# akamiru/bce

Hardware: AMD Instinct MI355X
Metric: MB/s compressed (higher is better)
Workload: dtype u8/u32 integer

## Files before the change

### bce_amd/csrc/api.hip

```cpp
#include <condition_variable>
#include <functional>
#include <mutex>
#include <thread>
#include <new>
#include <utility>

#include "bce_cost.h"
#include "common.h"
#include "host_coder.h"
#include "scan_coder.h"

#include <dlfcn.h>
#include <errno.h>
#include <fcntl.h>
#include <sys/file.h>
#include <sys/mman.h>
#include <sys/stat.h>
#include <unistd.h>

using namespace bce;

#ifndef K3_BATCH_MID
#define K3_BATCH_MID 8u
#endif
// ... 938 lines not shown
  c->stats.t_enum = c->stats.k3_ms * 1e-3;
  if (gate_timing)
    fprintf(stderr, "gate: ctx %p waited %.1f ms, held %.1f ms of %.1f ms from encode's start to its last flush queued (K3 %.1f ms, model %.1f ms, %llu flushes); coders' tail %.1f ms\n",
            (void *)c, c->gate_wait_s * 1e3, c->gate_held_s * 1e3, (t_gpu_done - t_enc0) * 1e3, c->stats.k3_ms, c->stats.t_model * 1e3,
            (unsigned long long)c->stats.flushes, (now_s() - t_gpu_done) * 1e3);
  return BCE_HIP_OK;
}

static int encode_body(bce_hip_ctx *c);
int bce_hip_encode(bce_hip_ctx *c) { return gate_on_error(c, bce_guarded(c, [&] { return encode_body(c); })); }
static int encode_body(bce_hip_ctx *c) {
  BCE_TRY(check_stage(c, 3));
  PhaseScope phase(c, 3);
  const double t_enc0 = now_s();
  BCE_TRY(encode_start(c));
  Enumeration e(c, [&](uint64_t nsym) { return flush_symbols(c, nsym); });
  BCE_TRY(e.run());
  return encode_end(c, e.ctl, t_enc0);
}

static bool early_enum_applies(const bce_hip_ctx *c) {
  const char *e = getenv("BCE_HIP_EARLY_ENUM");
  return !(e && e[0] == '0' && !e[1]) && k1_two_halves(c);
}
static uint32_t early_round_limit(uint32_t h) {
  uint32_t limit = 8u * h;
  if (const char *e = getenv("BCE_HIP_EARLY_CAP")) { const unsigned long v = strtoul(e, nullptr, 10); if (v < limit) limit = (uint32_t)v; }
  return limit;
}
static int compress_early_body(bce_hip_ctx *c) {
  BCE_TRY(check_stage(c, 1));
  BCE_HIP_TRY(c, hipSetDevice(c->device));
  c->stage = 1; c->enum_active = false;
  uint32_t h = 0;
  double t0 = now_s();
  PhaseScope phase(c, 1);
  {
    RoctxRange range("bce K1 first sort + provisional BWT");
    BCE_TRY(k1_first_sort(c, &h));
    BCE_TRY(k1_provisional_bwt(c));
  }
  double t_bwt = now_s() - t0;
  t0 = now_s();
  phase.set(2);
  {
    RoctxRange range("bce K2 planes + rank directory (provisional)");
    BCE_TRY(k2_build_planes(c));
  }
  double t_planes = now_s() - t0;
  uint32_t zeros0[8];
  memcpy(zeros0, c->zeros, sizeof zeros0);

  phase.set(6);
  const double t_enc0 = now_s();
  BCE_TRY(encode_start(c));
  Enumeration e(c, [&](uint64_t nsym) { return flush_symbols(c, nsym); });
  e.round_limit = early_round_limit(h);
  BCE_TRY(e.run());
  if (!e.paused) { gate_release(c); c->gate_lent = false; }
  const uint32_t paused_at = c->round;
  const uint64_t early_syms = c->stats.symbols;
  const double t_early = now_s() - t_enc0;

  t0 = now_s();
  {
    RoctxRange range("bce K1 second half + BWT");
    BCE_TRY(k1_finish(c));
    BCE_TRY(k1_final_bwt(c, c->k1_first_final));
  }
  t_bwt += now_s() - t0;
  if (!c->k1_first_final) {
    t0 = now_s();
    RoctxRange range("bce K2 planes + rank directory");
    BCE_TRY(k2_build_planes(c));
    t_planes += now_s() - t0;
    if (memcmp(zeros0, c->zeros, sizeof zeros0) != 0) {
      snprintf(c->err, sizeof c->err, "early rounds: the planes of the provisional and of the final BWT differ in their zero counts");
      return BCE_HIP_E_INTERNAL;
    }
  }
  c->stats.t_bwt = t_bwt;
  c->stats.t_planes = t_planes;
  if (getenv("BCE_HIP_EARLY_TRACE"))
    fprintf(stderr, "early: h %u limit %u %s at round %u (%s) symbols %llu rounds %.2f ms k1_finish+planes %.2f ms first_sort_final %d\n", h, e.round_limit,
            e.paused ? "paused" : "finished", paused_at, !e.paused ? "end" : (paused_at >= e.round_limit ? "limit" : "tail due"),
            (unsigned long long)early_syms, t_early * 1e3, (now_s() - t_enc0 - t_early) * 1e3, (int)c->k1_first_final);
  phase.set(3);
  if (e.paused) {
    e.round_limit = Enumeration::kNoLimit;
    BCE_TRY(e.run());
  }
  return encode_end(c, e.ctl, t_enc0);
}
static int compress_early(bce_hip_ctx *c) {
  const int rc = gate_on_error(c, bce_guarded(c, [&] { return compress_early_body(c); }));
  if (rc != BCE_HIP_OK && c) { c->stage = c->text_loaded ? 1 : 0; c->enum_active = false; c->k1_valid = false; }
  return rc;
}

static int scan_body(bce_hip_ctx *c, uint8_t *config288, double *result_bytes);
int bce_hip_scan(bce_hip_ctx *c, uint8_t config288[BCE_HIP_CONFIG_BYTES], double result_bytes[9]) {
  const int r = bce_guarded(c, [&] { return scan_body(c, config288, result_bytes); });
  if (c) gate_release(c);
  return r;
}
static int scan_body(bce_hip_ctx *c, uint8_t *config288, double *result_bytes) {
  BCE_TRY(check_stage(c, 3));
  if (!config288) return BCE_HIP_E_ARG;
  const double t_begin = now_s();
  gate_acquire(c);
  BCE_HIP_TRY(c, hipSetDevice(c->device));
  c->coder->drain();
  c->scan_mode = true;
  PhaseScope phase(c, 3);
  struct Reset { bce_hip_ctx *c; ~Reset() { c->scan_mode = false; } } reset{c};
  BCE_TRY(k4_prepare(c));
  BCE_TRY(k3_begin(c));
  c->stats.t_coder = 0;
  ScanSet coders;
  struct PinnedWords {
    uint32_t *p = nullptr; size_t cap = 0;
    ~PinnedWords() { if (p) (void)hipHostFree(p); }
    int ensure(size_t words) {
      if (words <= cap) return 0;
      if (p) { (void)hipHostFree(p); p = nullptr; cap = 0; }
      if (hipHostMalloc(reinterpret_cast<void **>(&p), words * 4, hipHostMallocDefault) != hipSuccess) { p = nullptr; return 1; }
      cap = words;
      return 0;
    }
  } host;
  double t_copy = 0, t_record = 0, t_pin = 0;
  auto consume = [&](uint64_t nsym) -> int {
    if (nsym) {
      const double tp0 = now_s();
      if (host.ensure((size_t)nsym > (size_t)c->sym_cap ? (size_t)nsym : (size_t)c->sym_cap)) return BCE_HIP_E_NOMEM;
      const double tc0 = now_s();
      t_pin += tc0 - tp0;
      BCE_HIP_TRY(c, hipMemcpyAsync(host.p, c->scanrec.p, (size_t)nsym * 4, hipMemcpyDeviceToHost, c->stream));
      BCE_HIP_TRY(c, hipStreamSynchronize(c->stream));
      t_copy += now_s() - tc0;
      std::vector<ScanSpan> spans[8];
      for (int p = 0; p < 8; ++p)
        for (const RunEntry &e : c->run_log[p]) spans[p].push_back(ScanSpan{e.start, e.count});
      const double t0 = now_s();
      coders.consume(host.p, spans);
      c->stats.t_coder += now_s() - t0;
      t_record += now_s() - t0;
    }
    return k3_reset_symbols(c);
  };
  c->stats.flushes = 0; c->stats.symbols = 0;
  Enumeration e(c, [&](uint64_t nsym) { c->stats.flushes++; c->stats.symbols += nsym; return consume(nsym); });
  BCE_TRY(e.run());
  c->stats.rounds = e.ctl.done_round;
  c->stats.nodes = e.ctl.nodes_total;
  c->enum_active = false;
  uint8_t init[9][32];
  memset(init, 0, sizeof init);
  double res[9];
  const double tf0 = now_s();
  coders.flush(init, res);
  c->stats.t_coder += now_s() - tf0;
  if (getenv("BCE_HIP_SCAN_DEBUG"))
    fprintf(stderr, "scan: %llu symbols in %llu batches: pinned buffer %.3f s, device-to-host copies %.3f s, recording %.3f s, optimisation %.3f s on %u host threads; K3 %.1f ms; %.3f s since entry\n",
            (unsigned long long)c->stats.symbols, (unsigned long long)c->stats.flushes, t_pin, t_copy, t_record, now_s() - tf0, coders.threads(), c->stats.k3_ms, now_s() - t_begin);
  if (result_bytes) memcpy(result_bytes, res, sizeof res);
  memcpy(config288, init, BCE_HIP_CONFIG_BYTES);
  if (getenv("BCE_HIP_SCAN_DEBUG")) {
    const double t0 = now_s();
// ... 291 lines not shown
```

### bce_amd/csrc/common.h

```cpp
#pragma once
#include <hip/hip_runtime.h>
#include <stdint.h>
#include <stdio.h>
#include <stdlib.h>
#include <string.h>

#include <atomic>
#include <chrono>
#include <condition_variable>
#include <exception>
#include <new>
#include <memory>
#include <mutex>
#include <thread>
#include <vector>

#include <sys/mman.h>

#include "../../include/bce_hip.h"
#include "bce_core.h"
#include "host_coder.h"

namespace bce {

// ... 51 lines not shown
  if (base == MAP_FAILED) return nullptr;
  char *q = reinterpret_cast<char *>((reinterpret_cast<uintptr_t>(base) + two_mb - 1) & ~(uintptr_t)(two_mb - 1));
  const size_t head = (size_t)(q - static_cast<char *>(base));
  if (head) (void)munmap(base, head);
  if (two_mb - head) (void)munmap(q + used, two_mb - head);
  (void)madvise(q, used, MADV_DONTFORK);
  static const bool no_thp = getenv("BCE_HIP_NO_THP") != nullptr;
  if (!no_thp) (void)madvise(q, used, MADV_HUGEPAGE);
  return q;
}
inline void reg_map_settle(void *q, size_t bytes) { (void)madvise(q, (bytes + 4095) & ~(size_t)4095, MADV_NOHUGEPAGE); }
inline void huge_unmap(void *q, size_t bytes) { if (q) (void)munmap(q, (bytes + 4095) & ~(size_t)4095); }
inline size_t slot_map_bytes(size_t cap) { return (cap * 8 + 16 + 4095) & ~(size_t)4095; }
inline void slot_free_host(FlushSlot &s, uint32_t *unmaps = nullptr) {
  if (s.h_out) {
    if (s.registered) {
      if (s.ev_copy) (void)hipEventSynchronize(s.ev_copy);
      (void)hipHostUnregister(s.h_out);
      huge_unmap(s.h_out, slot_map_bytes(s.cap));
      if (unmaps) ++*unmaps;
    } else (void)hipHostFree(s.h_out);
  }
  s.h_out = nullptr; s.cap = 0; s.registered = false;
}

struct RunEntry { uint64_t start; uint32_t count; uint32_t round; };

namespace qb {
enum Id {
  cnt_res,
  cnt_pat, cnt_off, cnt_out,
  loc_res,
  loc_lo, loc_cnt, loc_drop, loc_start, loc_lin, loc_bsum,
  loc_key0, loc_key1, loc_val0, loc_val1,
  loc_pat, loc_off, loc_hits, loc_pos,
  mat_res,
  mat_bsum,
  mat_qry, mat_len, mat_pos,
  rep_res,
  rep_bsum,
  rep_lcp,
  par_res,
  par_exit, par_entry, par_flag,
  par_bsum, par_bcnt,
  par_hpre,
  par_off, par_loff,
  par_ops, par_lits, par_out,
  count
};
}

}

struct bce_hip_ctx {
  int device = 0;
  hipStream_t stream = nullptr;
  hipStream_t copy_stream = nullptr;
  hipStream_t k4_stream = nullptr;
  hipEvent_t ev_k3_batch = nullptr;
  hipEvent_t ev_k4_done[2] = {nullptr, nullptr};
  bool overlap = false;
  bool gated = true;
  bool gate_held = false;
  bool gate_lent = false;
  double gate_t0 = 0, gate_wait_s = 0, gate_held_s = 0;
  uint32_t flush_seq = 0;
  hipEvent_t copy_busy = nullptr;
  hipEvent_t ev0 = nullptr, ev1 = nullptr, ev_k4 = nullptr;
  char err[256] = {0};

  uint32_t n = 0;
  int stage = 0;
  int phase = 0;
  uint32_t offset = 0;
  uint8_t config[9][32];
  bce::PlaneCfg cfg[8];
  uint32_t zeros[8] = {0};
  bool k1_unique = false;
  bool k1_valid = false;
  int sa_res = 0;
  int k1_res = 0;
  uint32_t k1_h = 0;
  bool k1_first_final = false;
  uint32_t dbg_dfs_budget = 0, dbg_no_dfs = 0, dbg_no_tail = 0, dbg_no_skip = 0, dbg_no_small = 0, dbg_step_small = 0, dbg_no_fused = 0, dbg_no_local = 0, dbg_capp_div = 0, dbg_local_from = 0, dbg_local_budget = 0, dbg_tail_round = 0;
  uint32_t dbg_dec_budget = 0;
  uint32_t dbg_oom = 0;
  uint64_t sym_cap_user = 0;
  bool sync_flush = false;
  bce_hip_progress_fn progress = nullptr;
  void *progress_user = nullptr;

  bce::DevBuf text, bwt;
  bce::DevBuf sa[2], key[2], rank, k2, nrk, act[2];
  bce::DevBuf khi[2], dl[4], kflag, actv[2];
  bce::DevBuf rs_hist, blk;
  bce::DevBuf ptmp[2];
  bce::DevBuf gran;
  uint32_t ngran = 0;
  bce::DevBuf nlist[2];
  uint32_t capL[2] = {0, 0};
  bce::DevBuf dlist[2][8];
  int dec_part = 0;
  bce::DevBuf ctl, tilecnt, tileoff, runs;
  bce::DevBuf smwords;
  size_t k3_groups = 0;
  uint32_t k3_count2_grid = 0;
  bce::DevBuf k3tw, k3grp;
  bce::DevBuf dfs;
  bce::DevBuf truns;
  void *h_truns = nullptr;
  bce::DevBuf skey[2], sval[2], sout, sesc;
  bce::DevBuf skey_alt, sesc_alt, rs_hist_k4;
  uint64_t sym_cap = 0;
  bool estimate_mode = false;
  bool scan_mode = false;
  bce::DevBuf scanrec;
  bce::DevBuf stat, dcfg, k4w;
  bce::DevBuf cost_acc, cost_runs;
  bce::DevBuf crc_tab;
  uint32_t crc_tab_grid = 0;
  bce::DevBuf cmp_res;
  bce::DevBuf qbuf[bce::qb::count];
  bce::DevBuf hook[3];
  bool crc_const_ready = false;
  bool text_loaded = false;
  uint32_t stat_off[8] = {0};
  bool model_hook = false;

  void *h_ctl = nullptr, *h_runs = nullptr;
  void *h_small = nullptr;
  void *h_big = nullptr;
  size_t h_big_cap = 0;
  uint32_t dec_restarts = 0;
  uint64_t dec_list_grows = 0, dec_split_rounds = 0;
  uint32_t reg_maps = 0, reg_unmaps = 0;
  bool h_big_registered = false;
  void *dec_pin[3] = {nullptr, nullptr, nullptr};
  size_t dec_pin_cap[3] = {0, 0, 0};
  bce::FlushSlot slot[3];
  int slot_next = 0;

  uint32_t round = 0;
  bool enum_active = false;
  std::vector<bce::RunEntry> run_log[8];

  bce::HostCoder *coder = nullptr;
  bce_hip_stats stats;
  std::mutex stage_mu;
  std::condition_variable stage_cv;
  int stage_state = 1;
  double alloc_s = 0, pin_s = 0;
  uint64_t alloc_bytes = 0, pin_bytes = 0;
  uint32_t alloc_calls = 0, pin_calls = 0;
};

namespace bce {

inline double now_s() {
  return std::chrono::duration<double>(std::chrono::steady_clock::now().time_since_epoch()).count();
}

void *big_host_alloc(size_t bytes, int device, bool *registered);
void big_host_free(bce_hip_ctx *c, void *p, size_t bytes, bool registered);

inline int set_err(bce_hip_ctx *c, hipError_t e, const char *what, int line) {
  snprintf(c->err, sizeof c->err, "%s:%d: %s", what, line, hipGetErrorString(e));
// ... 187 lines not shown
```

### bce_amd/csrc/k1_bwt.hip

```cpp
#include <stdlib.h>

#include <utility>

#include "common.h"
#include "scan_util.h"

namespace bce {

#ifndef K1_ACT_TENTHS
#define K1_ACT_TENTHS 6
#endif

constexpr int K1_T = 256;

constexpr uint32_t K1_MAXB = 1024;
struct K1Plan { uint32_t nb, per_block; };
static K1Plan k1_plan(uint32_t n) {
  const uint32_t chunk = 2048;
  uint32_t chunks = (uint32_t)(((uint64_t)n + chunk - 1) / chunk);
  if (!chunks) chunks = 1;
  uint32_t nb = chunks < K1_MAXB ? chunks : K1_MAXB;
  uint32_t cpb = (chunks + nb - 1) / nb;
  nb = (chunks + cpb - 1) / cpb;
  return {nb, cpb * chunk};
// ... 283 lines not shown
  auto rerank = [&](const uint32_t *k1s, const uint32_t *k2s, const uint32_t *sa) -> int {
    BCE_HIP_TRY(c, hipMemsetAsync(scalars, 0, 4, c->stream));
    hipLaunchKernelGGL(k1_heads_kernel, dim3(pl.nb), dim3(K1_T), 0, c->stream, k1s, k2s, n, pl.per_block, nrk,
                       blockmax, scalars);
    hipLaunchKernelGGL(k1_apply_kernel, dim3(pl.nb), dim3(K1_T), 0, c->stream, nrk, blockmax, n, pl.per_block, sa,
                       rank);
    BCE_TRY(read_back(c, &groups, scalars, 4));
    return BCE_HIP_OK;
  };
  BCE_TRY(rerank(key[res], nullptr, val[res]));
  const uint32_t bits = ceil_log2(n);
  const uint32_t dg = 9;
  uint64_t h = sentinel ? 3 : 4;
  uint32_t *act[2] = {c->act[0].as<uint32_t>(), c->act[1].as<uint32_t>()};
  uint32_t m = n;
  bool have_list = false;
  auto build_active = [&](const uint32_t *nrk_in, const uint32_t *src, uint32_t cnt, uint32_t *out) -> int {
    const K1Plan ap = k1_plan(cnt);
    hipLaunchKernelGGL(k1_active_kernel<0>, dim3(ap.nb), dim3(K1_T), 0, c->stream, nrk_in, src, cnt, ap.per_block, ap.nb,
                       blockmax, out, scalars + 2);
    hipLaunchKernelGGL(k1_active_kernel<1>, dim3(ap.nb), dim3(K1_T), 0, c->stream, nrk_in, src, cnt, ap.per_block, ap.nb,
                       blockmax, out, scalars + 2);
    BCE_TRY(read_back(c, &m, scalars + 2, 4));
    return BCE_HIP_OK;
  };
  const bool trace = getenv("BCE_K1_TRACE") != nullptr;
  double t_prev = now_s();
  if (trace) fprintf(stderr, "k1 %p: start n %u groups %u\n", (void *)c, n, groups);
  while (groups < n && h < n) {
    if (trace) { const double t = now_s(); fprintf(stderr, "k1 %p: h %llu groups %u m %u list %d (+%.2f ms)\n", (void *)c, (unsigned long long)h, groups, m, (int)have_list, (t - t_prev) * 1e3); t_prev = t; }
    if (!have_list && (uint64_t)(n - groups) * 10 < (uint64_t)n * K1_ACT_TENTHS + 10) {
      BCE_TRY(build_active(nrk, nullptr, n, act[0]));
      have_list = true;
      if (m == 0) break;
    }
    if (have_list && (uint64_t)m * 10 < (uint64_t)n * K1_ACT_TENTHS) {
      const uint32_t *A = act[0];
      uint32_t *ki[2] = {key[0], key[1]};
      uint32_t *vi[2] = {val[res ^ 1], k2};
      const uint32_t ga = grid_for(m);
      hipLaunchKernelGGL(k1_act_gather_kernel, dim3(ga), dim3(K1_T), 0, c->stream, A, val[res], rank, n, m, (uint32_t)h,
                         ki[0], vi[0]);
      int r1 = 0;
      BCE_TRY(radix_sort_pairs(c, ki, vi, m, 0, bits, &r1, dg));
      uint32_t *kj[2] = {ki[r1 ^ 1], ki[r1]};
      uint32_t *vj[2] = {vi[r1], vi[r1 ^ 1]};
      hipLaunchKernelGGL(k1_act_group_kernel, dim3(ga), dim3(K1_T), 0, c->stream, vj[0], rank, m, kj[0]);
      int r2 = 0;
      BCE_TRY(radix_sort_pairs(c, kj, vj, m, 0, bits, &r2, dg));
      const K1Plan ap = k1_plan(m);
      hipLaunchKernelGGL(k1_act_heads_kernel, dim3(ap.nb), dim3(K1_T), 0, c->stream, A, vj[r2], kj[r2], rank, n, m,
                         (uint32_t)h, ap.per_block, val[res], nrk, blockmax);
      hipLaunchKernelGGL(k1_act_apply_kernel, dim3(ap.nb), dim3(K1_T), 0, c->stream, nrk, blockmax, m, ap.per_block,
                         vj[r2], rank);
      BCE_TRY(build_active(nrk, A, m, act[1]));
      std::swap(act[0], act[1]);
      h <<= 1;
      c->stats.sort_rounds++;
      if (m == 0) break;
      continue;
    }
    uint32_t *ki[2] = {key[res ^ 1], key[res]};
    uint32_t *vi[2] = {val[res ^ 1], val[res]};
    hipLaunchKernelGGL(k1_gather_prev_kernel, dim3(g), dim3(K1_T), 0, c->stream, val[res], rank, n, (uint32_t)h,
                       ki[0], vi[0]);
    int r2 = 0;
    BCE_TRY(radix_sort_pairs(c, ki, vi, n, 0, bits, &r2, dg));
    uint32_t *sk = ki[r2], *ssa = vi[r2];
    hipLaunchKernelGGL(k1_gather_next_kernel, dim3(g), dim3(K1_T), 0, c->stream, ssa, rank, n, (uint32_t)h, k2);
    BCE_TRY(rerank(sk, k2, ssa));
    res = (ssa == val[0]) ? 0 : 1;
    h <<= 1;
    c->stats.sort_rounds++;
    have_list = false;
  }
  c->k1_unique = (groups >= n) || (have_list && m == 0);
  c->sa_res = res;
  return BCE_HIP_OK;
}


constexpr uint32_t K1_SLOT = 0x7FFFFFFFu, K1_HEAD = 0x80000000u;
constexpr uint32_t K1_SC_HIST = 16, K1_SC_CODE = 16 + 256;
constexpr uint8_t KF_HEAD = 1, KF_KEEP = 2, KF_DEFER = 4;

__global__ __launch_bounds__(K1_T) void k1_bytehist_kernel(const uint8_t *__restrict__ T, uint32_t n, uint32_t *__restrict__ hist) {
  __shared__ uint32_t lh[256];
  lh[threadIdx.x] = 0;
  __syncthreads();
  for (uint64_t i = (uint64_t)blockIdx.x * K1_T + threadIdx.x; i < n; i += (uint64_t)gridDim.x * K1_T) atomicAdd(&lh[T[i]], 1u);
  __syncthreads();
  if (lh[threadIdx.x]) atomicAdd(&hist[threadIdx.x], lh[threadIdx.x]);
}

constexpr int K1I_E = 8;
__global__ __launch_bounds__(K1_T) void k1_init64_kernel(const uint8_t *__restrict__ T, uint32_t m, uint32_t nbytes,
                                                         const uint16_t *__restrict__ code, uint32_t bits, uint32_t nsym,
                                                         uint32_t *__restrict__ lo, uint32_t *__restrict__ hi, uint32_t *__restrict__ val) {
  __shared__ uint16_t sym[K1_T * K1I_E + 16];
  __shared__ uint16_t lut[256];
  lut[threadIdx.x] = code[threadIdx.x];
  __syncthreads();
  const uint64_t base = (uint64_t)blockIdx.x * (K1_T * K1I_E);
  for (uint32_t i = threadIdx.x; i < K1_T * K1I_E + 16; i += K1_T) {
    uint64_t q = base + i;
    if (q >= m) q %= m;
    sym[i] = q < nbytes ? lut[T[q]] : (uint16_t)0;
  }
  __syncthreads();
#pragma unroll
  for (int e = 0; e < K1I_E; ++e) {
    const uint32_t o = (uint32_t)e * K1_T + threadIdx.x;
    const uint64_t p = base + o;
    if (p < m) {
      uint64_t k = 0;
      for (uint32_t b = 0; b < nsym; ++b) k = (k << bits) | sym[o + b];
      lo[p] = (uint32_t)k;
      hi[p] = (uint32_t)(k >> 32);
      val[p] = (uint32_t)p;
    }
  }
}

constexpr int SEG_T = 1024;
constexpr int SEG_CH = 2048;
constexpr int SEG_CAP = 2048;
constexpr int SEG_W = SEG_CH + SEG_CAP;
constexpr int SEG_HW = SEG_W + SEG_CAP;

__device__ __forceinline__ int seg_prev_bit(const uint64_t *b, int pos, int lo_limit) {
  int wi = pos >> 6;
  uint64_t word = b[wi] & (~0ull >> (63 - (pos & 63)));
  const int wl = lo_limit >> 6;
  while (word == 0 && wi > wl) { --wi; word = b[wi]; }
  if (!word) return -1;
  const int r = wi * 64 + 63 - __clzll((long long)word);
  return r >= lo_limit ? r : -1;
}
__device__ __forceinline__ int seg_next_bit(const uint64_t *b, int pos, int hi_limit) {
  int wi = pos >> 6;
  uint64_t word = (pos & 63) == 63 ? 0ull : (b[wi] & (~0ull << ((pos & 63) + 1)));
  const int wh = hi_limit >> 6;
  while (word == 0 && wi < wh) { ++wi; word = b[wi]; }
  if (!word) return -1;
  const int r = wi * 64 + __ffsll((long long)word) - 1;
  return r <= hi_limit ? r : -1;
}

__global__ __launch_bounds__(SEG_T) void k1_seg_sort_kernel(const uint32_t *__restrict__ A, const uint32_t *__restrict__ V, uint32_t m, uint32_t *__restrict__ sa,
                                                            const uint32_t *__restrict__ rank, uint32_t n, uint32_t h,
                                                            uint32_t *__restrict__ nr, uint32_t *__restrict__ vs,
                                                            uint8_t *__restrict__ flag, uint32_t *__restrict__ ndefer) {
  __shared__ uint64_t hb[SEG_HW / 64 + 1];
  __shared__ uint64_t nbits[SEG_W / 64 + 1];
  __shared__ __attribute__((aligned(16))) uint32_t K[SEG_W];
  __shared__ uint32_t S[SEG_W], SL[SEG_W];
  __shared__ uint32_t s_defer;
  __shared__ int s_cntw;
  const uint32_t tid = threadIdx.x, lane = tid & 63u;
  const int64_t base = (int64_t)blockIdx.x * SEG_CH;
  if (tid == 0) { s_defer = 0; hb[SEG_HW / 64] = 0; nbits[SEG_W / 64] = 0; }
#pragma unroll
  for (int it = 0; it < SEG_HW / SEG_T; ++it) {
    const int u = it * SEG_T + (int)tid;
    const int64_t i = base - SEG_CAP + u;
    uint32_t a = 0;
    bool hd = false;
    if (i >= 0) {
      if (i < (int64_t)m) { a = A[i]; hd = (a & K1_HEAD) != 0u; }
      else hd = true;
    }
    const uint64_t bal = __ballot(hd);
    if (lane == 0) hb[u >> 6] = bal;
    if (u >= SEG_CAP) SL[u - SEG_CAP] = a & K1_SLOT;
  }
  __syncthreads();
  if (tid == 0) {
    const int e = seg_next_bit(hb, SEG_CAP + SEG_CH - 1, SEG_HW - 1);
    const int cw = (e < 0 ? SEG_HW : e) - SEG_CAP;
    s_cntw = cw > SEG_CH ? cw : SEG_CH;
  }
  __syncthreads();
  const int cntw = s_cntw;
  constexpr int EPT = SEG_W / SEG_T;
  uint32_t k2[EPT], sfx[EPT];
  int gs[EPT], ge[EPT];
  bool mine[EPT];
  uint32_t ndef = 0;
#pragma unroll
  for (int it = 0; it < EPT; ++it) {
    const int w = it * SEG_T + (int)tid, u = w + SEG_CAP;
    const int64_t i = base + w;
    mine[it] = false; gs[it] = 0; ge[it] = 0; k2[it] = 0; sfx[it] = 0;
    if (w < cntw && i < (int64_t)m) {
      const int g0 = seg_prev_bit(hb, u, u - SEG_CAP + 1);
      bool big = g0 < 0;
      int g1 = -1;
      if (!big) {
        const int lim = g0 + SEG_CAP < SEG_HW - 1 ? g0 + SEG_CAP : SEG_HW - 1;
        g1 = seg_next_bit(hb, u, lim);
        big = g1 < 0;
      }
      if (big) {
// ... 137 lines not shown
      hbase += htot;
    }
  }
}

__global__ __launch_bounds__(K1_T) void k1_big_gather_kernel(const uint32_t *__restrict__ idx, const uint32_t *__restrict__ gid,
                                                             const uint32_t *__restrict__ V, const uint32_t *__restrict__ rank,
                                                             uint32_t n, uint32_t nd, uint32_t h, uint32_t rbits,
                                                             uint32_t *__restrict__ lo, uint32_t *__restrict__ hi, uint32_t *__restrict__ val) {
  for (uint64_t j = (uint64_t)blockIdx.x * K1_T + threadIdx.x; j < nd; j += (uint64_t)gridDim.x * K1_T) {
    const uint32_t p = V[idx[j]];
    uint64_t q = (uint64_t)p + h;
    if (q >= n) q -= n;
    const uint64_t key = ((uint64_t)gid[j] << rbits) | rank[q];
    lo[j] = (uint32_t)key;
    hi[j] = (uint32_t)(key >> 32);
    val[j] = p;
  }
}
__global__ __launch_bounds__(K1_T) void k1_big_heads_kernel(const uint32_t *__restrict__ slots, const uint32_t *__restrict__ lo,
                                                            const uint32_t *__restrict__ hi, const uint32_t *__restrict__ val,
                                                            uint32_t nd, uint32_t per_block, uint32_t *__restrict__ sa,
                                                            uint32_t *__restrict__ nrk, uint32_t *__restrict__ blockmax) {
  const uint64_t beg = (uint64_t)blockIdx.x * per_block;
  uint64_t end = beg + per_block;
  if (end > nd) end = nd;
  uint32_t mx = 0;
  for (uint64_t j = beg + threadIdx.x; j < end; j += K1_T) {
    const uint32_t slot = slots[j];
    sa[slot] = val[j];
    const bool head = j == 0 || lo[j] != lo[j - 1] || hi[j] != hi[j - 1];
    nrk[j] = head ? slot : 0u;
    if (head) mx = slot;
  }
  mx = block_reduce_max<K1_T>(mx);
  if (threadIdx.x == 0) blockmax[blockIdx.x] = mx;
}

__global__ __launch_bounds__(K1_T) void k1_defer_flags_kernel(const uint32_t *__restrict__ nrk, const uint32_t *__restrict__ idx,
                                                              const uint32_t *__restrict__ sorted, uint32_t nd,
                                                              uint8_t *__restrict__ flag, uint32_t *__restrict__ vs) {
  for (uint64_t j = (uint64_t)blockIdx.x * K1_T + threadIdx.x; j < nd; j += (uint64_t)gridDim.x * K1_T) {
    const bool hd = j == 0 || nrk[j] != 0u;
    const bool nx = j + 1 >= nd || nrk[j + 1] != 0u;
    const uint32_t i = idx[j];
    flag[i] = (uint8_t)(KF_DEFER | (hd ? KF_HEAD : 0) | ((hd && nx) ? 0 : KF_KEEP));
    vs[i] = sorted[j];
  }
}

static uint32_t k1_part_min() {
  static const uint32_t part_min = getenv("BCE_K1_PART_MIN") ? (uint32_t)strtoul(getenv("BCE_K1_PART_MIN"), nullptr, 10) : K1_PART_MIN;
  return part_min;
}

struct K1View {
  bce_hip_ctx *c;
  uint32_t n, g;
  K1Plan pl;
  uint32_t *blockmax, *scalars;
  uint32_t *rank, *k2, *nrk;
  uint8_t *flag;
  uint32_t *lo[2], *hi[2], *val[2];
  bool trace;
  double t_prev;
  explicit K1View(bce_hip_ctx *ctx, uint32_t n_) : c(ctx), n(n_), g(grid_for(n_)), pl(k1_plan(n_)) {
    blockmax = c->blk.as<uint32_t>();
    scalars = blockmax + K1_MAXB;
    rank = c->rank.as<uint32_t>(); k2 = c->k2.as<uint32_t>(); nrk = c->nrk.as<uint32_t>();
    flag = c->kflag.as<uint8_t>();
    for (int i = 0; i < 2; ++i) { lo[i] = c->key[i].as<uint32_t>(); hi[i] = c->khi[i].as<uint32_t>(); val[i] = c->sa[i].as<uint32_t>(); }
    trace = getenv("BCE_K1_TRACE") != nullptr;
    t_prev = now_s();
  }
  void lap(const char *what, uint64_t h, uint32_t m, uint32_t nd) {
    if (!trace) return;
    (void)hipStreamSynchronize(c->stream);
    const double t = now_s();
    fprintf(stderr, "k1 %p: %-10s h %llu active %u deferred %u (+%.2f ms)\n", (void *)c, what, (unsigned long long)h, m, nd, (t - t_prev) * 1e3);
    t_prev = t;
  }
};

static int k1_first_sort_wide(bce_hip_ctx *c, const uint8_t *T, uint32_t n, bool sentinel) {
  const size_t b4 = (size_t)n * 4;
  for (int i = 0; i < 2; ++i) { BCE_TRY(ensure(c, c->sa[i], b4)); BCE_TRY(ensure(c, c->key[i], b4)); BCE_TRY(ensure(c, c->khi[i], b4)); }
  BCE_TRY(ensure(c, c->rank, b4));
  BCE_TRY(ensure(c, c->k2, b4));
  BCE_TRY(ensure(c, c->nrk, b4));
  BCE_TRY(ensure(c, c->kflag, (size_t)n + 16));
  for (int i = 0; i < 2; ++i) { BCE_TRY(ensure(c, c->act[i], b4)); BCE_TRY(ensure(c, c->actv[i], b4)); }
  BCE_TRY(ensure(c, c->blk, (size_t)(K1_MAXB + K1_SC_CODE + 128 + K1_MAXB) * 4));
  K1View v(c, n);
  uint32_t *const scalars = v.scalars;
  const uint32_t g = v.g;

  const uint32_t nbytes = sentinel ? n - 1u : n;
  BCE_HIP_TRY(c, hipMemsetAsync(scalars + K1_SC_HIST, 0, 256 * 4, c->stream));
  hipLaunchKernelGGL(k1_bytehist_kernel, dim3(g < 1024u ? g : 1024u), dim3(K1_T), 0, c->stream, T, nbytes, scalars + K1_SC_HIST);
  uint32_t hist[256];
  BCE_TRY(read_back(c, hist, scalars + K1_SC_HIST, sizeof hist));
  uint16_t code[256];
  uint32_t sigma = sentinel ? 1u : 0u;
  for (int b = 0; b < 256; ++b) { code[b] = (uint16_t)sigma; if (hist[b]) ++sigma; }
  uint32_t bits = ceil_log2(sigma);
  if (bits < 1) bits = 1;
  uint32_t nsym = 64u / bits;
  if (nsym > 16u) nsym = 16u;
  if (const char *e = getenv("BCE_K1_KEYBITS")) { const uint32_t kb = (uint32_t)strtoul(e, nullptr, 10); if (kb >= bits && kb / bits < nsym) nsym = kb / bits; }
  const uint32_t keybits = nsym * bits;
  {
    if (!c->h_small) BCE_TRY(pin_alloc(c, &c->h_small, 4096));
    memcpy(c->h_small, code, sizeof code);
    BCE_HIP_TRY(c, hipMemcpyAsync(scalars + K1_SC_CODE, c->h_small, sizeof code, hipMemcpyHostToDevice, c->stream));
  }

  {
    const uint32_t per = K1_T * K1I_E;
    hipLaunchKernelGGL(k1_init64_kernel, dim3((uint32_t)(((uint64_t)n + per - 1) / per)), dim3(K1_T), 0, c->stream, T, n, nbytes,
                       reinterpret_cast<const uint16_t *>(scalars + K1_SC_CODE), bits, nsym, v.lo[0], v.hi[0], v.val[0]);
  }
  int res = 0;
  BCE_TRY(radix_sort_wide(c, v.lo, v.hi, v.val, n, keybits, &res, 9));
  v.lap("first sort", nsym, n, 0);
  BCE_HIP_TRY(c, hipGetLastError());
  c->k1_res = res;
  c->k1_h = nsym;
  return BCE_HIP_OK;
}

static int k1_finish_wide(bce_hip_ctx *c, uint32_t n) {
  K1View v(c, n);
  const K1Plan pl = v.pl;
  uint32_t *const blockmax = v.blockmax, *const scalars = v.scalars, *const rank = v.rank, *const k2 = v.k2, *const nrk = v.nrk;
  uint8_t *const flag = v.flag;
  uint32_t **const lo = v.lo, **const hi = v.hi, **const val = v.val;
  const uint32_t g = v.g;
  (void)g;
  const int res = c->k1_res;
  const uint32_t nsym = c->k1_h;
  auto lap = [&](const char *what, uint64_t h, uint32_t m, uint32_t nd) { v.lap(what, h, m, nd); };
  BCE_HIP_TRY(c, hipMemsetAsync(scalars, 0, 16, c->stream));
  hipLaunchKernelGGL(k1_heads_kernel, dim3(pl.nb), dim3(K1_T), 0, c->stream, hi[res], lo[res], n, pl.per_block, nrk, blockmax, scalars);
  const uint32_t rbits = ceil_log2(n);
  const uint32_t part_min = k1_part_min();
  const bool sorted_apply = n >= part_min;
  if (sorted_apply) hipLaunchKernelGGL(k1_headidx_kernel, dim3(pl.nb), dim3(K1_T), 0, c->stream, nrk, blockmax, n, pl.per_block, k2);
  else hipLaunchKernelGGL(k1_apply_kernel, dim3(pl.nb), dim3(K1_T), 0, c->stream, nrk, blockmax, n, pl.per_block, val[res], rank);
  uint32_t *act[2] = {c->act[0].as<uint32_t>(), c->act[1].as<uint32_t>()};
  uint32_t *actv[2] = {c->actv[0].as<uint32_t>(), c->actv[1].as<uint32_t>()};
  uint32_t m = 0;
  hipLaunchKernelGGL(k1_active_kernel<0>, dim3(pl.nb), dim3(K1_T), 0, c->stream, nrk, (const uint32_t *)nullptr, n, pl.per_block, pl.nb,
                     blockmax, act[0], scalars + 2, 1u, (const uint32_t *)val[res], actv[0]);
  hipLaunchKernelGGL(k1_active_kernel<1>, dim3(pl.nb), dim3(K1_T), 0, c->stream, nrk, (const uint32_t *)nullptr, n, pl.per_block, pl.nb,
                     blockmax, act[0], scalars + 2, 1u, (const uint32_t *)val[res], actv[0]);
  if (sorted_apply) {
    const uint32_t b1 = rbits / ((rbits + 9u) / 10u);
    uint32_t *pk[2] = {val[res], lo[res ^ 1]}, *pv[2] = {k2, rank};
    int pr = 0;
    BCE_TRY(radix_sort_pairs(c, pk, pv, n, 0, b1, &pr, 10));
    uint32_t *qk[2] = {lo[res ^ 1], hi[res ^ 1]}, *qv[2] = {rank, val[res ^ 1]};
    BCE_TRY(radix_sort_pairs(c, qk, qv, n, b1, rbits - b1, &pr, 10));
    if (pr) BCE_HIP_TRY(c, hipMemcpyAsync(rank, qv[1], (size_t)n * 4, hipMemcpyDeviceToDevice, c->stream));
  }
  BCE_TRY(read_back(c, &m, scalars + 2, 4));
  lap("first ranks", nsym, m, 0);
  c->k1_first_final = m == 0 || nsym >= n;

  uint64_t h = nsym;
  uint32_t *sa = val[res];
  uint32_t *nr = hi[0], *vs = hi[1];
  while (m > 0 && h < n) {
    const uint32_t *A = act[0];
    const uint32_t nblk = (uint32_t)(((uint64_t)m + SEG_CH - 1) / SEG_CH);
    BCE_HIP_TRY(c, hipMemsetAsync(scalars + 3, 0, 4, c->stream));
    hipLaunchKernelGGL(k1_seg_sort_kernel, dim3(nblk), dim3(SEG_T), 0, c->stream, A, (const uint32_t *)actv[0], m, sa, rank, n, (uint32_t)h, nr, vs,
                       flag, scalars + 3);
    uint32_t nd = 0;
    BCE_TRY(read_back(c, &nd, scalars + 3, 4));
    const K1Plan ap = k1_plan(m);
    if (nd) {
      BCE_TRY(ensure(c, c->dl[0], (size_t)nd * 4));
      BCE_TRY(ensure(c, c->dl[1], (size_t)nd * 4));
      BCE_TRY(ensure(c, c->dl[2], (size_t)nd * 4));
      BCE_TRY(ensure(c, c->dl[3], (size_t)nd * 4));
      uint32_t *idx = c->dl[0].as<uint32_t>(), *slots = c->dl[1].as<uint32_t>(), *gid = c->dl[2].as<uint32_t>();
      uint32_t *blockcnt2 = scalars + K1_SC_CODE + 128;
      hipLaunchKernelGGL((k1_relist_kernel<0, 0>), dim3(ap.nb), dim3(K1_T), 0, c->stream, A, (const uint32_t *)vs, flag, m, ap.per_block, ap.nb, blockmax, idx, slots,
                         scalars + 4, blockcnt2, gid);
      hipLaunchKernelGGL((k1_relist_kernel<1, 0>), dim3(ap.nb), dim3(K1_T), 0, c->stream, A, (const uint32_t *)vs, flag, m, ap.per_block, ap.nb, blockmax, idx, slots,
                         scalars + 4, blockcnt2, gid);
      uint32_t cnts[2] = {0, 0};
      BCE_TRY(read_back(c, cnts, scalars + 4, 8));
      if (cnts[0] != nd || cnts[1] == 0 || cnts[1] > nd) { snprintf(c->err, sizeof c->err, "k1: deferred list %u / %u groups, expected %u elements", cnts[0], cnts[1], nd); return BCE_HIP_E_INTERNAL; }
      const uint32_t gbits = ceil_log2(cnts[1]);
      uint32_t *bl[2] = {lo[0], lo[1]};
      uint32_t *bh[2] = {val[res ^ 1], k2};
      uint32_t *bv[2] = {nrk, c->dl[3].as<uint32_t>()};
      const uint32_t ga = grid_for(nd);
      hipLaunchKernelGGL(k1_big_gather_kernel, dim3(ga), dim3(K1_T), 0, c->stream, idx, gid, (const uint32_t *)actv[0], rank, n, nd, (uint32_t)h, rbits,
                         bl[0], bh[0], bv[0]);
      int rb = 0;
      BCE_TRY(radix_sort_wide(c, bl, bh, bv, nd, rbits + gbits, &rb, 9));
      const K1Plan dp = k1_plan(nd);
      uint32_t *snrk = bv[rb ^ 1];
      hipLaunchKernelGGL(k1_big_heads_kernel, dim3(dp.nb), dim3(K1_T), 0, c->stream, slots, bl[rb], bh[rb], bv[rb], nd, dp.per_block, sa, snrk, blockmax);
      hipLaunchKernelGGL(k1_act_apply_kernel, dim3(dp.nb), dim3(K1_T), 0, c->stream, snrk, blockmax, nd, dp.per_block, bv[rb], rank);
      uint32_t *vjr = bv[rb];
      hipLaunchKernelGGL(k1_defer_flags_kernel, dim3(ga), dim3(K1_T), 0, c->stream, snrk, idx, (const uint32_t *)vjr, nd, flag, vs);
    }
    if (m >= part_min) {
      const uint32_t b1 = rbits / ((rbits + 9u) / 10u);
      uint32_t *pk[2] = {lo[0], lo[1]}, *pv[2] = {nr, k2};
      hipLaunchKernelGGL(k1_seg_pairs_kernel, dim3(grid_for(m)), dim3(K1_T), 0, c->stream, (const uint32_t *)vs, (const uint8_t *)flag, KF_DEFER, m, pk[0]);
      int pr = 0;
      BCE_TRY(radix_sort_pairs(c, pk, pv, m, 0, b1, &pr, 10));
      uint32_t *qk[2] = {lo[1], lo[0]}, *qv[2] = {k2, val[res ^ 1]};
      BCE_TRY(radix_sort_pairs(c, qk, qv, m, b1, rbits - b1, &pr, 10));
      hipLaunchKernelGGL(k1_scatter32_kernel, dim3(grid_for(m)), dim3(K1_T), 0, c->stream, (const uint32_t *)qk[pr], (const uint32_t *)qv[pr], m, n, rank);
    } else {
      hipLaunchKernelGGL(k1_seg_apply_kernel, dim3(grid_for(m)), dim3(K1_T), 0, c->stream, nr, vs, flag, m, rank);
    }
    hipLaunchKernelGGL((k1_relist_kernel<0, 1>), dim3(ap.nb), dim3(K1_T), 0, c->stream, A, (const uint32_t *)vs, flag, m, ap.per_block, ap.nb, blockmax, act[1],
                       actv[1], scalars + 2);
    hipLaunchKernelGGL((k1_relist_kernel<1, 1>), dim3(ap.nb), dim3(K1_T), 0, c->stream, A, (const uint32_t *)vs, flag, m, ap.per_block, ap.nb, blockmax, act[1],
                       actv[1], scalars + 2);
    const uint32_t m_old = m;
    BCE_TRY(read_back(c, &m, scalars + 2, 4));
    std::swap(act[0], act[1]);
    std::swap(actv[0], actv[1]);
    h <<= 1;
    c->stats.sort_rounds++;
    lap("round", h, m, nd);
    (void)m_old;
  }
  BCE_HIP_TRY(c, hipGetLastError());
  c->k1_unique = m == 0;
  c->sa_res = res;
  return BCE_HIP_OK;
}

static int k1_sort_rotations(bce_hip_ctx *c, const uint8_t *T, uint32_t n, bool sentinel) {
  if (getenv("BCE_K1_V1")) return k1_sort_rotations_v1(c, T, n, sentinel);
  BCE_TRY(k1_first_sort_wide(c, T, n, sentinel));
  return k1_finish_wide(c, n);
}

bool k1_two_halves(const bce_hip_ctx *c) {
  return c->n >= 2 && c->n < k1_part_min() && !getenv("BCE_K1_V1");
}

static int k1_begin(bce_hip_ctx *c) {
  BCE_TRY(ensure(c, c->bwt, c->n));
  c->stats.sort_rounds = 0;
  c->k1_unique = false;
  c->k1_valid = false;
  c->k1_first_final = false;
  return BCE_HIP_OK;
}

int k1_first_sort(bce_hip_ctx *c, uint32_t *h_symbols) {
  BCE_TRY(k1_begin(c));
  BCE_TRY(k1_first_sort_wide(c, c->text.as<uint8_t>(), c->n, false));
  if (h_symbols) *h_symbols = c->k1_h;
  return BCE_HIP_OK;
}

int k1_provisional_bwt(bce_hip_ctx *c) {
  const uint32_t n = c->n;
  hipLaunchKernelGGL(k1_bwt_kernel, dim3(grid_for(n)), dim3(K1_T), 0, c->stream, c->text.as<uint8_t>(), c->sa[c->k1_res].as<uint32_t>(), n,
                     c->bwt.as<uint8_t>());
  BCE_HIP_TRY(c, hipGetLastError());
  return BCE_HIP_OK;
}

int k1_finish(bce_hip_ctx *c) { return k1_finish_wide(c, c->n); }

int k1_final_bwt(bce_hip_ctx *c, bool have_bwt) {
  const uint32_t n = c->n;
  const uint32_t g = grid_for(n);
  uint32_t *scalars = c->blk.as<uint32_t>() + K1_MAXB;
  const uint32_t *sa = c->sa[c->sa_res].as<uint32_t>();
  BCE_HIP_TRY(c, hipMemsetAsync(scalars + 1, 0xFF, 4, c->stream));
  if (!have_bwt) hipLaunchKernelGGL(k1_bwt_kernel, dim3(g), dim3(K1_T), 0, c->stream, c->text.as<uint8_t>(), sa, n, c->bwt.as<uint8_t>());
  hipLaunchKernelGGL(k1_offset_kernel, dim3(g), dim3(K1_T), 0, c->stream, c->rank.as<uint32_t>(), n, scalars + 1);
  uint32_t off = 0;
  BCE_TRY(read_back(c, &off, scalars + 1, 4));
  BCE_HIP_TRY(c, hipGetLastError());
  if (off >= n) { snprintf(c->err, sizeof c->err, "k1: no rank-0 rotation found"); return BCE_HIP_E_INTERNAL; }
  c->offset = off;
  c->k1_valid = true;
  return BCE_HIP_OK;
}

int k1_bwt(bce_hip_ctx *c) {
  const uint32_t n = c->n;
  uint8_t *T = c->text.as<uint8_t>();
  BCE_TRY(k1_begin(c));
  if (n == 1) {
    BCE_HIP_TRY(c, hipMemcpyAsync(c->bwt.p, T, 1, hipMemcpyDeviceToDevice, c->stream));
    BCE_HIP_TRY(c, hipStreamSynchronize(c->stream));
    c->offset = 0;
    return BCE_HIP_OK;
  }
  BCE_TRY(k1_sort_rotations(c, T, n, false));
  return k1_final_bwt(c, false);
}

__global__ __launch_bounds__(K1_T) void k1_divbwt_gather_kernel(const uint8_t *__restrict__ T, const uint32_t *__restrict__ sa,
                                                                uint32_t m, uint32_t pidx, uint8_t *__restrict__ U) {
  for (uint64_t j = (uint64_t)blockIdx.x * K1_T + threadIdx.x; j < m; j += (uint64_t)gridDim.x * K1_T) {
    const uint32_t p = sa[j];
    if (p != 0u) U[j < pidx ? j : j - 1u] = T[p - 1u];
  }
}

int k1_divbwt(bce_hip_ctx *c, const uint8_t *T_host, uint8_t *U_host, uint32_t n, uint32_t *pidx_out) {
  if (n == 0 || n >= 0x7FFFFFFFu) return BCE_HIP_E_ARG;
  const uint32_t m = n + 1u;
  c->stage = 0; c->k1_valid = false; c->enum_active = false; c->text_loaded = false;
  BCE_TRY(ensure(c, c->text, m));
  BCE_TRY(ensure(c, c->bwt, m));
  uint8_t *T = c->text.as<uint8_t>();
  BCE_HIP_TRY(c, hipMemcpyAsync(T, T_host, n, hipMemcpyHostToDevice, c->stream));
  c->stats.sort_rounds = 0;
  BCE_TRY(k1_sort_rotations(c, T, m, true));
  uint32_t pidx = 0;
  BCE_TRY(read_back(c, &pidx, c->rank.as<uint32_t>(), 4));
  if (pidx == 0 || pidx > n) { snprintf(c->err, sizeof c->err, "divbwt: primary index %u out of range", pidx); return BCE_HIP_E_INTERNAL; }
  hipLaunchKernelGGL(k1_divbwt_gather_kernel, dim3(grid_for(m)), dim3(K1_T), 0, c->stream, T, c->sa[c->sa_res].as<uint32_t>(), m,
                     pidx, c->bwt.as<uint8_t>());
  BCE_HIP_TRY(c, hipMemcpyAsync(U_host, c->bwt.p, n, hipMemcpyDeviceToHost, c->stream));
  BCE_HIP_TRY(c, hipStreamSynchronize(c->stream));
  BCE_HIP_TRY(c, hipGetLastError());
  *pidx_out = pidx;
  return BCE_HIP_OK;
}

}
```

Before: 899.8.

## Carry preceding symbol in sort values to build provisional BWT without text gather

```diff
diff --git a/bce_amd/csrc/api.hip b/bce_amd/csrc/api.hip
--- a/bce_amd/csrc/api.hip
+++ b/bce_amd/csrc/api.hip
@@ -1044,9 +1044,10 @@
   c->stats.t_bwt = t_bwt;
   c->stats.t_planes = t_planes;
   if (getenv("BCE_HIP_EARLY_TRACE"))
-    fprintf(stderr, "early: h %u limit %u %s at round %u (%s) symbols %llu rounds %.2f ms k1_finish+planes %.2f ms first_sort_final %d\n", h, e.round_limit,
+    fprintf(stderr, "early: h %u limit %u %s at round %u (%s) symbols %llu rounds %.2f ms k1_finish+planes %.2f ms first_sort_final %d bwt %s\n", h, e.round_limit,
             e.paused ? "paused" : "finished", paused_at, !e.paused ? "end" : (paused_at >= e.round_limit ? "limit" : "tail due"),
-            (unsigned long long)early_syms, t_early * 1e3, (now_s() - t_enc0 - t_early) * 1e3, (int)c->k1_first_final);
+            (unsigned long long)early_syms, t_early * 1e3, (now_s() - t_enc0 - t_early) * 1e3, (int)c->k1_first_final,
+            c->k1_carried ? "carried" : "gathered");
   phase.set(3);
   if (e.paused) {
     e.round_limit = Enumeration::kNoLimit;
diff --git a/bce_amd/csrc/common.h b/bce_amd/csrc/common.h
--- a/bce_amd/csrc/common.h
+++ b/bce_amd/csrc/common.h
@@ -157,6 +157,8 @@
   int k1_res = 0;
   uint32_t k1_h = 0;
   bool k1_first_final = false;
+  uint32_t k1_pbits = 0;
+  bool k1_carried = false;
   uint32_t dbg_dfs_budget = 0, dbg_no_dfs = 0, dbg_no_tail = 0, dbg_no_skip = 0, dbg_no_small = 0, dbg_step_small = 0, dbg_no_fused = 0, dbg_no_local = 0, dbg_capp_div = 0, dbg_local_from = 0, dbg_local_budget = 0, dbg_tail_round = 0;
   uint32_t dbg_dec_budget = 0;
   uint32_t dbg_oom = 0;
diff --git a/bce_amd/csrc/k1_bwt.hip b/bce_amd/csrc/k1_bwt.hip
--- a/bce_amd/csrc/k1_bwt.hip
+++ b/bce_amd/csrc/k1_bwt.hip
@@ -389,6 +389,10 @@
 
 constexpr uint32_t K1_SLOT = 0x7FFFFFFFu, K1_HEAD = 0x80000000u;
 constexpr uint32_t K1_SC_HIST = 16, K1_SC_CODE = 16 + 256;
+constexpr uint32_t K1_SC_BYTE = K1_SC_CODE + 128;
+constexpr uint32_t K1_SC_CNT2 = K1_SC_BYTE + 64;
+constexpr uint32_t K1_SC_END = K1_SC_CNT2 + K1_MAXB;
+constexpr uint32_t K1_EARLY_BITS = 5, K1_EARLY_NSYM = 10, K1_EARLY_MIN_N = 1u << 20;
 constexpr uint8_t KF_HEAD = 1, KF_KEEP = 2, KF_DEFER = 4;
 
 __global__ __launch_bounds__(K1_T) void k1_bytehist_kernel(const uint8_t *__restrict__ T, uint32_t n, uint32_t *__restrict__ hist) {
@@ -402,15 +406,15 @@
 
 constexpr int K1I_E = 8;
 __global__ __launch_bounds__(K1_T) void k1_init64_kernel(const uint8_t *__restrict__ T, uint32_t m, uint32_t nbytes,
-                                                         const uint16_t *__restrict__ code, uint32_t bits, uint32_t nsym,
+                                                         const uint16_t *__restrict__ code, uint32_t bits, uint32_t nsym, uint32_t carry_at,
                                                          uint32_t *__restrict__ lo, uint32_t *__restrict__ hi, uint32_t *__restrict__ val) {
-  __shared__ uint16_t sym[K1_T * K1I_E + 16];
+  __shared__ uint16_t sym[K1_T * K1I_E + 17];
   __shared__ uint16_t lut[256];
   lut[threadIdx.x] = code[threadIdx.x];
   __syncthreads();
   const uint64_t base = (uint64_t)blockIdx.x * (K1_T * K1I_E);
-  for (uint32_t i = threadIdx.x; i < K1_T * K1I_E + 16; i += K1_T) {
-    uint64_t q = base + i;
+  for (uint32_t i = threadIdx.x; i < K1_T * K1I_E + 17; i += K1_T) {
+    uint64_t q = base + i + (m - 1u);
     if (q >= m) q %= m;
     sym[i] = q < nbytes ? lut[T[q]] : (uint16_t)0;
   }
@@ -421,11 +425,33 @@
     const uint64_t p = base + o;
     if (p < m) {
       uint64_t k = 0;
-      for (uint32_t b = 0; b < nsym; ++b) k = (k << bits) | sym[o + b];
+      for (uint32_t b = 0; b < nsym; ++b) k = (k << bits) | sym[o + 1u + b];
       lo[p] = (uint32_t)k;
       hi[p] = (uint32_t)(k >> 32);
-      val[p] = (uint32_t)p;
-    }
+      val[p] = (uint32_t)p | (carry_at ? (uint32_t)sym[o] << carry_at : 0u);
+    }
+  }
+}
+
+__global__ __launch_bounds__(K1_T) void k1_carried_bwt_kernel(uint32_t *__restrict__ val, uint32_t n, uint32_t carry_at,
+                                                              const uint8_t *__restrict__ byte_of, uint8_t *__restrict__ bwt) {
+  __shared__ uint8_t lut[256];
+  lut[threadIdx.x] = byte_of[threadIdx.x];
+  __syncthreads();
+  const uint32_t mask = (1u << carry_at) - 1u;
+  const uint32_t n4 = n / 4u;
+  uint4 *__restrict__ v4 = reinterpret_cast<uint4 *>(val);
+  uint32_t *__restrict__ b4 = reinterpret_cast<uint32_t *>(bwt);
+  for (uint64_t j = (uint64_t)blockIdx.x * K1_T + threadIdx.x; j < n4; j += (uint64_t)gridDim.x * K1_T) {
+    uint4 v = v4[j];
+    b4[j] = (uint32_t)lut[v.x >> carry_at] | (uint32_t)lut[v.y >> carry_at] << 8 | (uint32_t)lut[v.z >> carry_at] << 16 |
+            (uint32_t)lut[v.w >> carry_at] << 24;
+    v.x &= mask; v.y &= mask; v.z &= mask; v.w &= mask;
+    v4[j] = v;
+  }
+  if (blockIdx.x == 0) {
+    const uint32_t j = n4 * 4u + threadIdx.x;
+    if (j < n) { const uint32_t v = val[j]; bwt[j] = lut[v >> carry_at]; val[j] = v & mask; }
   }
 }
 
@@ -729,7 +755,7 @@
   }
 };
 
-static int k1_first_sort_wide(bce_hip_ctx *c, const uint8_t *T, uint32_t n, bool sentinel) {
+static int k1_first_sort_wide(bce_hip_ctx *c, const uint8_t *T, uint32_t n, bool sentinel, bool one_shot = false) {
   const size_t b4 = (size_t)n * 4;
   for (int i = 0; i < 2; ++i) { BCE_TRY(ensure(c, c->sa[i], b4)); BCE_TRY(ensure(c, c->key[i], b4)); BCE_TRY(ensure(c, c->khi[i], b4)); }
   BCE_TRY(ensure(c, c->rank, b4));
@@ -737,7 +763,7 @@
   BCE_TRY(ensure(c, c->nrk, b4));
   BCE_TRY(ensure(c, c->kflag, (size_t)n + 16));
   for (int i = 0; i < 2; ++i) { BCE_TRY(ensure(c, c->act[i], b4)); BCE_TRY(ensure(c, c->actv[i], b4)); }
-  BCE_TRY(ensure(c, c->blk, (size_t)(K1_MAXB + K1_SC_CODE + 128 + K1_MAXB) * 4));
+  BCE_TRY(ensure(c, c->blk, (size_t)(K1_MAXB + K1_SC_END) * 4));
   K1View v(c, n);
   uint32_t *const scalars = v.scalars;
   const uint32_t g = v.g;
@@ -748,24 +774,33 @@
   uint32_t hist[256];
   BCE_TRY(read_back(c, hist, scalars + K1_SC_HIST, sizeof hist));
   uint16_t code[256];
+  uint8_t byte_of[256] = {0};
   uint32_t sigma = sentinel ? 1u : 0u;
-  for (int b = 0; b < 256; ++b) { code[b] = (uint16_t)sigma; if (hist[b]) ++sigma; }
+  for (int b = 0; b < 256; ++b) { code[b] = (uint16_t)sigma; if (hist[b]) byte_of[sigma++ & 255u] = (uint8_t)b; }
   uint32_t bits = ceil_log2(sigma);
   if (bits < 1) bits = 1;
-  uint32_t nsym = 64u / bits;
-  if (nsym > 16u) nsym = 16u;
-  if (const char *e = getenv("BCE_K1_KEYBITS")) { const uint32_t kb = (uint32_t)strtoul(e, nullptr, 10); if (kb >= bits && kb / bits < nsym) nsym = kb / bits; }
+  uint32_t full = 64u / bits;
+  if (full > 16u) full = 16u;
+  uint32_t nsym = full;
+  if (one_shot && bits == K1_EARLY_BITS && n >= K1_EARLY_MIN_N && nsym > K1_EARLY_NSYM) nsym = K1_EARLY_NSYM;
+  if (const char *e = getenv("BCE_K1_KEYBITS")) { const uint32_t kb = (uint32_t)strtoul(e, nullptr, 10); if (kb >= bits) nsym = kb / bits < full ? kb / bits : full; }
   const uint32_t keybits = nsym * bits;
+  const uint32_t pbits = ceil_log2(n);
+  bool carry = one_shot;
+  if (carry) { const char *e = getenv("BCE_HIP_CARRY_BWT"); carry = !(e && e[0] == '0' && !e[1]); }
+  c->k1_pbits = carry && !sentinel && pbits >= 1 && bits + pbits <= 32 ? pbits : 0u;
   {
+    static_assert((K1_SC_BYTE - K1_SC_CODE) * 4 == sizeof code, "the byte table lies right behind the code table: one copy");
     if (!c->h_small) BCE_TRY(pin_alloc(c, &c->h_small, 4096));
     memcpy(c->h_small, code, sizeof code);
-    BCE_HIP_TRY(c, hipMemcpyAsync(scalars + K1_SC_CODE, c->h_small, sizeof code, hipMemcpyHostToDevice, c->stream));
+    memcpy(static_cast<uint8_t *>(c->h_small) + sizeof code, byte_of, sizeof byte_of);
+    BCE_HIP_TRY(c, hipMemcpyAsync(scalars + K1_SC_CODE, c->h_small, sizeof code + sizeof byte_of, hipMemcpyHostToDevice, c->stream));
   }
 
   {
     const uint32_t per = K1_T * K1I_E;
     hipLaunchKernelGGL(k1_init64_kernel, dim3((uint32_t)(((uint64_t)n + per - 1) / per)), dim3(K1_T), 0, c->stream, T, n, nbytes,
-                       reinterpret_cast<const uint16_t *>(scalars + K1_SC_CODE), bits, nsym, v.lo[0], v.hi[0], v.val[0]);
+                       reinterpret_cast<const uint16_t *>(scalars + K1_SC_CODE), bits, nsym, c->k1_pbits, v.lo[0], v.hi[0], v.val[0]);
   }
   int res = 0;
   BCE_TRY(radix_sort_wide(c, v.lo, v.hi, v.val, n, keybits, &res, 9));
@@ -786,6 +821,7 @@
   (void)g;
   const int res = c->k1_res;
   const uint32_t nsym = c->k1_h;
+  if (c->k1_pbits) { snprintf(c->err, sizeof c->err, "k1: the first sort's values still carry the preceding symbols"); return BCE_HIP_E_INTERNAL; }
   auto lap = [&](const char *what, uint64_t h, uint32_t m, uint32_t nd) { v.lap(what, h, m, nd); };
   BCE_HIP_TRY(c, hipMemsetAsync(scalars, 0, 16, c->stream));
   hipLaunchKernelGGL(k1_heads_kernel, dim3(pl.nb), dim3(K1_T), 0, c->stream, hi[res], lo[res], n, pl.per_block, nrk, blockmax, scalars);
@@ -832,7 +868,7 @@
       BCE_TRY(ensure(c, c->dl[2], (size_t)nd * 4));
       BCE_TRY(ensure(c, c->dl[3], (size_t)nd * 4));
       uint32_t *idx = c->dl[0].as<uint32_t>(), *slots = c->dl[1].as<uint32_t>(), *gid = c->dl[2].as<uint32_t>();
-      uint32_t *blockcnt2 = scalars + K1_SC_CODE + 128;
+      uint32_t *blockcnt2 = scalars + K1_SC_CNT2;
       hipLaunchKernelGGL((k1_relist_kernel<0, 0>), dim3(ap.nb), dim3(K1_T), 0, c->stream, A, (const uint32_t *)vs, flag, m, ap.per_block, ap.nb, blockmax, idx, slots,
                          scalars + 4, blockcnt2, gid);
       hipLaunchKernelGGL((k1_relist_kernel<1, 0>), dim3(ap.nb), dim3(K1_T), 0, c->stream, A, (const uint32_t *)vs, flag, m, ap.per_block, ap.nb, blockmax, idx, slots,
@@ -903,19 +939,27 @@
   c->k1_unique = false;
   c->k1_valid = false;
   c->k1_first_final = false;
+  c->k1_pbits = 0;
+  c->k1_carried = false;
   return BCE_HIP_OK;
 }
 
 int k1_first_sort(bce_hip_ctx *c, uint32_t *h_symbols) {
   BCE_TRY(k1_begin(c));
-  BCE_TRY(k1_first_sort_wide(c, c->text.as<uint8_t>(), c->n, false));
+  BCE_TRY(k1_first_sort_wide(c, c->text.as<uint8_t>(), c->n, false, true));
   if (h_symbols) *h_symbols = c->k1_h;
   return BCE_HIP_OK;
 }
 
 int k1_provisional_bwt(bce_hip_ctx *c) {
   const uint32_t n = c->n;
-  hipLaunchKernelGGL(k1_bwt_kernel, dim3(grid_for(n)), dim3(K1_T), 0, c->stream, c->text.as<uint8_t>(), c->sa[c->k1_res].as<uint32_t>(), n,
+  c->k1_carried = c->k1_pbits != 0;
+  if (c->k1_carried) {
+    const uint8_t *byte_of = reinterpret_cast<const uint8_t *>(c->blk.as<uint32_t>() + K1_MAXB + K1_SC_BYTE);
+    hipLaunchKernelGGL(k1_carried_bwt_kernel, dim3(grid_for(n / 4u)), dim3(K1_T), 0, c->stream, c->sa[c->k1_res].as<uint32_t>(), n, c->k1_pbits,
+                       byte_of, c->bwt.as<uint8_t>());
+    c->k1_pbits = 0;
+  } else hipLaunchKernelGGL(k1_bwt_kernel, dim3(grid_for(n)), dim3(K1_T), 0, c->stream, c->text.as<uint8_t>(), c->sa[c->k1_res].as<uint32_t>(), n,
                      c->bwt.as<uint8_t>());
   BCE_HIP_TRY(c, hipGetLastError());
   return BCE_HIP_OK;
```

Result: faster. 918.8 (median of 6 runs) (+2.1%).
